# HKPolyU-UAV/FLVIS

Hardware: AMD Instinct MI355X
Metric: frames/sec/node (640×480 stereo+IMU) + ATE vs CPU ref, EuRoC MH_05 (higher is better)
Workload: dtype u8/f32 LK+GFTT, f64 geometry+BA

## Files before the change

flvis_amd/csrc/lk_kernel.hip:

```cpp
#include "dev_common.hpp"
#include "img_kernels.hpp"

namespace flvis {

constexpr int LK_WIN = 31;
constexpr int LK_PS = 40;
constexpr int LK_PROWS = 34;
constexpr int LK_RM = 4;
constexpr int LK_RS = 52;
constexpr int LK_RROWS = 33 + 2 * LK_RM;
constexpr int LK_TC_HDR = 64;
constexpr int LK_TC_LVL = 64 * 24;

typedef short lk_s2 __attribute__((ext_vector_type(2)));
typedef __attribute__((address_space(1))) uint32_t lk_gu32;
typedef uint32_t lk_u4 __attribute__((ext_vector_type(4)));
__device__ __forceinline__ lk_s2 lk_as_s2(uint32_t v) { return __builtin_bit_cast(lk_s2, v); }
__device__ __forceinline__ float lk_uniform(float v) {
  return __builtin_bit_cast(float, __builtin_amdgcn_readfirstlane(__builtin_bit_cast(int, v)));
}
__device__ __forceinline__ long long lk_uniform64(long long v) {
  const uint32_t lo = (uint32_t)__builtin_amdgcn_readfirstlane((int)(uint32_t)v), hi = (uint32_t)__builtin_amdgcn_readfirstlane((int)(v >> 32));
  return (long long)(((unsigned long long)hi << 32) | lo);
}
typedef unsigned short lk_u2 __attribute__((ext_vector_type(2)));
template <int S>
__device__ __forceinline__ lk_s2 lk_pack_shr(int a0, int a1) {
  static_assert(S >= 8 && S <= 16, "bytes 1 and 2 hold bits 8 .. 23");
  const lk_u2 p = __builtin_bit_cast(lk_u2, __builtin_amdgcn_perm((uint32_t)a1, (uint32_t)a0, 0x06050201u));
  return __builtin_bit_cast(lk_s2, (lk_u2)(p >> (unsigned short)(S - 8)));
}

__device__ __forceinline__ bool lk_load_patch(const uint8_t* __restrict__ img, int w, int h, int pitch, int bx, int by, int X0, int Y0,
                                              int nrows, uint8_t* patch) {
  if (X0 >= -bx && Y0 >= -by && X0 + 39 < w + bx && Y0 + nrows <= h + by) {
    const lk_gu32* const base = (const lk_gu32*)(img + (ptrdiff_t)Y0 * pitch + (X0 & ~3));
    const int sh = X0 & 3;
    int r = (int)threadIdx.x / 9, k = (int)threadIdx.x - 9 * r;
    unsigned off = (unsigned)(r * pitch + 4 * k);
    static_assert(LK_PROWS * 9 <= 5 * 64, "five trips");
    const int n = nrows * 9;
    uint32_t lo[5], hi[5];
#pragma unroll
    for (int t = 0; t < 5; t++) {
      const bool on = (int)threadIdx.x + 64 * t < n;
      const unsigned o = on ? off : 0u;
      lo[t] = *(const lk_gu32*)((const __attribute__((address_space(1))) uint8_t*)base + o);
      hi[t] = *(const lk_gu32*)((const __attribute__((address_space(1))) uint8_t*)base + o + 4);
      k += 1;
      const bool wrap = k >= 9;
      k = wrap ? k - 9 : k;
      off += (unsigned)(7 * pitch + 4) + (wrap ? (unsigned)(pitch - 36) : 0u);
    }
#pragma unroll
    for (int t = 0; t < 5; t++) asm volatile("" : "+v"(lo[t]), "+v"(hi[t]));
    r = (int)threadIdx.x / 9;
    k = (int)threadIdx.x - 9 * r;
    unsigned dst = (unsigned)(r * LK_PS + 4 * k);
#pragma unroll
    for (int t = 0; t < 5; t++) {
      if ((int)threadIdx.x + 64 * t < n) *reinterpret_cast<uint32_t*>(patch + dst) = __builtin_amdgcn_alignbyte(hi[t], lo[t], sh);
      k += 1;
      const bool wrap = k >= 9;
      k = wrap ? k - 9 : k;
      dst += (unsigned)(7 * LK_PS + 4) + (wrap ? (unsigned)(LK_PS - 36) : 0u);
    }
    return false;
  }
  for (int i = threadIdx.x; i < nrows * 9; i += 64) {
    int r = i / 9, k = i - r * 9;
    int Y = Y0 + r, X = X0 + 4 * k;
    uint32_t v;
    if (Y >= 0 && Y < h && X >= 0 && X + 3 < w) {
      const uint8_t* row = img + (size_t)Y * pitch;
      int a = X & ~3, sh = X & 3;
      uint32_t lo = *reinterpret_cast<const uint32_t*>(row + a);
      uint32_t hi = sh ? *reinterpret_cast<const uint32_t*>(row + a + 4) : 0u;
      v = __builtin_amdgcn_alignbyte(hi, lo, sh);
    } else {
      const uint8_t* row = img + (size_t)reflect101c(Y, h) * pitch;
      uint32_t b0 = row[reflect101c(X, w)], b1 = row[reflect101c(X + 1, w)], b2 = row[reflect101c(X + 2, w)],
               b3 = row[reflect101c(X + 3, w)];
      v = b0 | (b1 << 8) | (b2 << 16) | (b3 << 24);
    }
    *reinterpret_cast<uint32_t*>(patch + r * LK_PS + 4 * k) = v;
  }
  return true;
}

__device__ __forceinline__ bool lk_load_region(const uint8_t* __restrict__ img, int w, int h, int pitch, int bx, int by, int X0, int Y0,
                                               uint8_t* region) {
  if (X0 >= -bx && Y0 >= -by && X0 + 51 < w + bx && Y0 + LK_RROWS <= h + by) {
    const __attribute__((address_space(1))) uint8_t* const base = (const __attribute__((address_space(1))) uint8_t*)(img + (ptrdiff_t)Y0 * pitch + X0);
    int r = (int)threadIdx.x / 13, k = (int)threadIdx.x - 13 * r;
    unsigned off = (unsigned)(r * pitch + 4 * k);
    static_assert(LK_RS == 52, "the region rows are contiguous in LDS: item i sits at byte 4 i");
    constexpr int N = LK_RROWS * 13, T = (N + 63) / 64;
    uint32_t v[T];
#pragma unroll
    for (int t = 0; t < T; t++) {
      const bool on = 64 * (t + 1) <= N || (int)threadIdx.x + 64 * t < N;
      v[t] = *(const lk_gu32*)(base + (on ? off : 0u));
      k += 12;
      const bool wrap = k >= 13;
      k = wrap ? k - 13 : k;
      off += (unsigned)(4 * pitch + 48) + (wrap ? (unsigned)(pitch - 52) : 0u);
    }
#pragma unroll
    for (int t = 0; t < T; t++) asm volatile("" : "+v"(v[t]));
#pragma unroll
    for (int t = 0; t < T; t++)
      if (64 * (t + 1) <= N || (int)threadIdx.x + 64 * t < N) *reinterpret_cast<uint32_t*>(region + 4 * ((int)threadIdx.x + 64 * t)) = v[t];
    return false;
  }
  for (int i = threadIdx.x; i < LK_RROWS * 13; i += 64) {
    int r = i / 13, k = i - r * 13;
    int Y = Y0 + r, X = X0 + 4 * k;
    uint32_t v;
    if (Y >= 0 && Y < h && X >= 0 && X + 3 < w) {
      v = *reinterpret_cast<const uint32_t*>(img + (size_t)Y * pitch + X);
    } else {
      const uint8_t* row = img + (size_t)reflect101c(Y, h) * pitch;
      uint32_t b0 = row[reflect101c(X, w)], b1 = row[reflect101c(X + 1, w)], b2 = row[reflect101c(X + 2, w)],
               b3 = row[reflect101c(X + 3, w)];
      v = b0 | (b1 << 8) | (b2 << 16) | (b3 << 24);
    }
    *reinterpret_cast<uint32_t*>(region + r * LK_RS + 4 * k) = v;
  }
  return true;
}

#define LK_PAIR(D, K)                                                                                              \
  ((((K)&3) == 3) ? __builtin_amdgcn_perm((D)[((K) >> 2) + 1], (D)[(K) >> 2], 0x0c040c03u)                         \
                  : __builtin_amdgcn_perm(0u, (D)[(K) >> 2], 0x0c000c00u | (uint32_t)((K)&3) | ((uint32_t)(((K)&3) + 1) << 16)))

__device__ __forceinline__ int lk_dot2_bias(lk_s2 a, lk_s2 b, int bias_uniform) {
  int r;
  asm("v_dot2_i32_i16 %0, %1, %2, %3" : "=v"(r) : "v"(a), "v"(b), "s"(bias_uniform));
  return r;
}
__device__ __forceinline__ void lk_wave_sum2_f32(int v1, int v2, float& f1, float& f2) {
  int a = v1 & 0xffff, b = v1 >> 16, c = v2 & 0xffff, d = v2 >> 16;
#define LK_STEP4(CTRL, RM)                                           \
  {                                                                  \
    const int ta = __builtin_amdgcn_update_dpp(0, a, CTRL, RM, 0xf, false); \
    const int tb = __builtin_amdgcn_update_dpp(0, b, CTRL, RM, 0xf, false); \
    const int tc = __builtin_amdgcn_update_dpp(0, c, CTRL, RM, 0xf, false); \
    const int td = __builtin_amdgcn_update_dpp(0, d, CTRL, RM, 0xf, false); \
    a += ta, b += tb, c += tc, d += td;                              \
  }
  LK_STEP4(0xB1, 0xf)
  LK_STEP4(0x4E, 0xf)
  LK_STEP4(0x141, 0xf)
  LK_STEP4(0x140, 0xf)
  LK_STEP4(0x142, 0xa)
  LK_STEP4(0x143, 0xc)
#undef LK_STEP4
  const float g1 = (float)__builtin_fma((double)b, 65536.0, (double)a), g2 = (float)__builtin_fma((double)d, 65536.0, (double)c);
  f1 = __builtin_bit_cast(float, __builtin_amdgcn_readlane(__builtin_bit_cast(int, g1), 63));
  f2 = __builtin_bit_cast(float, __builtin_amdgcn_readlane(__builtin_bit_cast(int, g2), 63));
}

__device__ __forceinline__ void lk_wave_sum3_wide(int v1, int v2, int v3, long long& s1, long long& s2, long long& s3) {
  int a = v1 & 0xffff, b = v1 >> 16, c = v2 & 0xffff, d = v2 >> 16, e = v3 & 0xffff, f = v3 >> 16;
#define LK_STEP6(CTRL, RM)                                                    \
  {                                                                           \
    const int ta = __builtin_amdgcn_update_dpp(0, a, CTRL, RM, 0xf, false);  \
    const int tb = __builtin_amdgcn_update_dpp(0, b, CTRL, RM, 0xf, false);  \
    const int tc = __builtin_amdgcn_update_dpp(0, c, CTRL, RM, 0xf, false);  \
    const int td = __builtin_amdgcn_update_dpp(0, d, CTRL, RM, 0xf, false);  \
    const int te = __builtin_amdgcn_update_dpp(0, e, CTRL, RM, 0xf, false);  \
    const int tf = __builtin_amdgcn_update_dpp(0, f, CTRL, RM, 0xf, false);  \
    a += ta, b += tb, c += tc, d += td, e += te, f += tf;                     \
  }
  LK_STEP6(0xB1, 0xf)
  LK_STEP6(0x4E, 0xf)
  LK_STEP6(0x141, 0xf)
  LK_STEP6(0x140, 0xf)
  LK_STEP6(0x142, 0xa)
  LK_STEP6(0x143, 0xc)
#undef LK_STEP6
  s1 = ((long long)__builtin_amdgcn_readlane(b, 63) << 16) + (long long)__builtin_amdgcn_readlane(a, 63);
  s2 = ((long long)__builtin_amdgcn_readlane(d, 63) << 16) + (long long)__builtin_amdgcn_readlane(c, 63);
  s3 = ((long long)__builtin_amdgcn_readlane(f, 63) << 16) + (long long)__builtin_amdgcn_readlane(e, 63);
}

template <bool INTERIOR>
__device__ __forceinline__ void lk_template(const uint8_t* patch, int lane, int ipx, int ipy, int W, int H, lk_s2 wT, lk_s2 wB,
                                            lk_s2 (&tI)[8], lk_s2 (&tX)[8], lk_s2 (&tY)[8], int& a11, int& a12, int& a22) {
  constexpr int W_BITS = 14;
  const int r = lane >> 1, c0 = (lane & 1) * 16;
  uint32_t d[3][5];
#pragma unroll
  for (int j = 0; j < 3; j++)
#pragma unroll
    for (int k = 0; k < 5; k++) d[j][k] = *reinterpret_cast<const uint32_t*>(patch + (r + j) * LK_PS + c0 + 4 * k);
  uint32_t bits = 0;
  if (!INTERIOR) {
    const int xs = ipx + c0, Y = ipy + r;
    int lo = -xs, hi = W - xs;
    lo = lo < 0 ? 0 : (lo > 18 ? 18 : lo);
    hi = hi < 0 ? 0 : (hi > 18 ? 18 : hi);
    bits = (Y >= 0 && Y < H && hi > lo) ? (((1u << hi) - 1u) & ~((1u << lo) - 1u)) : 0u;
  }
  lk_s2 DX[2][9], DY[2][9];
  {
    lk_s2 T0[10], T1[10];
#pragma unroll
    for (int j = 0; j < 10; j++) {
      const lk_s2 A = __builtin_bit_cast(lk_s2, LK_PAIR(d[0], 2 * j)), B = __builtin_bit_cast(lk_s2, LK_PAIR(d[1], 2 * j)),
                  Cc = __builtin_bit_cast(lk_s2, LK_PAIR(d[2], 2 * j));
      T0[j] = (A + Cc) * (short)3 + B * (short)10;
      T1[j] = Cc - A;
    }
    const int up2 = ((lane + 2) & 63) * 4;
#pragma unroll
    for (int j = 0; j < 9; j++) {
      DX[0][j] = T0[j + 1] - T0[j];
      const lk_s2 T1o = __builtin_bit_cast(lk_s2, __builtin_amdgcn_perm(__builtin_bit_cast(uint32_t, T1[j + 1]),
                                                                       __builtin_bit_cast(uint32_t, T1[j]), 0x05040302u));
      DY[0][j] = (T1[j + 1] + T1[j]) * (short)3 + T1o * (short)10;
      if (!INTERIOR) {
        const uint32_t m = ((bits >> (2 * j)) & 1u ? 0x0000ffffu : 0u) | ((bits >> (2 * j + 1)) & 1u ? 0xffff0000u : 0u);
        DX[0][j] = __builtin_bit_cast(lk_s2, __builtin_bit_cast(uint32_t, DX[0][j]) & m);
        DY[0][j] = __builtin_bit_cast(lk_s2, __builtin_bit_cast(uint32_t, DY[0][j]) & m);
      }
      DX[1][j] = __builtin_bit_cast(lk_s2, __builtin_amdgcn_ds_bpermute(up2, __builtin_bit_cast(int, DX[0][j])));
      DY[1][j] = __builtin_bit_cast(lk_s2, __builtin_amdgcn_ds_bpermute(up2, __builtin_bit_cast(int, DY[0][j])));
    }
  }
  if (r < LK_WIN) {
#pragma unroll
    for (int c2 = 0; c2 < 8; c2++) {
      int iv[2], ix[2], iy[2];
#pragma unroll
      for (int hh = 0; hh < 2; hh++) {
        const int c = 2 * c2 + hh;
        lk_s2 x0, x1, y0, y1;
        if (hh == 0) {
          x0 = DX[0][c2]; x1 = DX[1][c2]; y0 = DY[0][c2]; y1 = DY[1][c2];
        } else {
          x0 = __builtin_bit_cast(lk_s2, __builtin_amdgcn_perm(__builtin_bit_cast(uint32_t, DX[0][c2 + 1]), __builtin_bit_cast(uint32_t, DX[0][c2]), 0x05040302u));
          x1 = __builtin_bit_cast(lk_s2, __builtin_amdgcn_perm(__builtin_bit_cast(uint32_t, DX[1][c2 + 1]), __builtin_bit_cast(uint32_t, DX[1][c2]), 0x05040302u));
          y0 = __builtin_bit_cast(lk_s2, __builtin_amdgcn_perm(__builtin_bit_cast(uint32_t, DY[0][c2 + 1]), __builtin_bit_cast(uint32_t, DY[0][c2]), 0x05040302u));
          y1 = __builtin_bit_cast(lk_s2, __builtin_amdgcn_perm(__builtin_bit_cast(uint32_t, DY[1][c2 + 1]), __builtin_bit_cast(uint32_t, DY[1][c2]), 0x05040302u));
        }
        int ax = lk_dot2_bias(x0, wT, 1 << (W_BITS - 1)), ay = lk_dot2_bias(y0, wT, 1 << (W_BITS - 1));
        int ai = lk_dot2_bias(__builtin_bit_cast(lk_s2, LK_PAIR(d[1], c + 1)), wT, 1 << (W_BITS - 5 - 1));
        ax = __builtin_amdgcn_sdot2(x1, wB, ax, false);
        ay = __builtin_amdgcn_sdot2(y1, wB, ay, false);
        ai = __builtin_amdgcn_sdot2(__builtin_bit_cast(lk_s2, LK_PAIR(d[2], c + 1)), wB, ai, false);
        const bool on = c0 + c < LK_WIN;
        ix[hh] = on ? (ax >> W_BITS) : 0;
        iy[hh] = on ? (ay >> W_BITS) : 0;
        iv[hh] = on ? (ai >> (W_BITS - 5)) : 0;
      }
      tI[c2] = __builtin_bit_cast(lk_s2, __builtin_amdgcn_perm((uint32_t)iv[1], (uint32_t)iv[0], 0x05040100u));
      tX[c2] = __builtin_bit_cast(lk_s2, __builtin_amdgcn_perm((uint32_t)ix[1], (uint32_t)ix[0], 0x05040100u));
      tY[c2] = __builtin_bit_cast(lk_s2, __builtin_amdgcn_perm((uint32_t)iy[1], (uint32_t)iy[0], 0x05040100u));
      a11 = __builtin_amdgcn_sdot2(tX[c2], tX[c2], a11, false);
      a12 = __builtin_amdgcn_sdot2(tX[c2], tY[c2], a12, false);
      a22 = __builtin_amdgcn_sdot2(tY[c2], tY[c2], a22, false);
    }
  } else {
#pragma unroll
    for (int c = 0; c < 8; c++) {
      tI[c] = lk_s2{0, 0};
      tX[c] = lk_s2{0, 0};
      tY[c] = lk_s2{0, 0};
    }
  }
}

__device__ __forceinline__ bool lk_template_level(const uint8_t* img, int W, int H, int pitch, int bx, int by, int ipx, int ipy, int iw00,
                                                  int iw01, int iw10, int iw11, uint8_t* patch, int lane, lk_s2 (&tI)[8], lk_s2 (&tX)[8],
                                                  lk_s2 (&tY)[8], long long& iA11, long long& iA12, long long& iA22) {
  __syncthreads();
  const bool slow = lk_load_patch(img, W, H, pitch, bx, by, ipx - 1, ipy - 1, LK_PROWS, patch);
  __syncthreads();
  int a11 = 0, a12 = 0, a22 = 0;
  const bool interior = ipx >= 0 && ipx + 32 <= W - 1 && ipy >= 0 && ipy + 31 <= H - 1;
  const lk_s2 wT = lk_s2{(short)iw00, (short)iw01}, wB = lk_s2{(short)iw10, (short)iw11};
  if (interior)
    lk_template<true>(patch, lane, ipx, ipy, W, H, wT, wB, tI, tX, tY, a11, a12, a22);
  else
    lk_template<false>(patch, lane, ipx, ipy, W, H, wT, wB, tI, tX, tY, a11, a12, a22);
  lk_wave_sum3_wide(a11, a12, a22, iA11, iA12, iA22);
  return slow;
}
struct LKTmpl {
  uint32_t w[24];
  long long a11, a12, a22;
};
__device__ __noinline__ void lk_template_level_cold(const uint8_t* img, int W, int H, int pitch, int bx, int by, int ipx, int ipy, int iw00,
                                                    int iw01, int iw10, int iw11, uint8_t* patch, int lane, LKTmpl* out) {
  lk_s2 tI[8], tX[8], tY[8];
  long long a11, a12, a22;
  lk_template_level(img, W, H, pitch, bx, by, ipx, ipy, iw00, iw01, iw10, iw11, patch, lane, tI, tX, tY, a11, a12, a22);
#pragma unroll
  for (int k = 0; k < 8; k++) {
    out->w[k] = __builtin_bit_cast(uint32_t, tI[k]);
    out->w[8 + k] = __builtin_bit_cast(uint32_t, tX[k]);
    out->w[16 + k] = __builtin_bit_cast(uint32_t, tY[k]);
  }
  out->a11 = a11;
  out->a12 = a12;
  out->a22 = a22;
}

__device__ __forceinline__ void lk_tc_store_level(uint32_t* tc_ptr, int level, int lane, const lk_s2 (&tI)[8], const lk_s2 (&tX)[8],
                                                  const lk_s2 (&tY)[8], long long iA11, long long iA12, long long iA22) {
  lk_u4* dst = reinterpret_cast<lk_u4*>(tc_ptr + LK_TC_HDR + (size_t)level * LK_TC_LVL) + lane;
  uint32_t wI[8];
#pragma unroll
  for (int k = 0; k < 8; k++) wI[k] = __builtin_bit_cast(uint32_t, tI[k]);
  if (lane == 63) {
    wI[0] = (uint32_t)iA11; wI[1] = (uint32_t)((unsigned long long)iA11 >> 32);
    wI[2] = (uint32_t)iA12; wI[3] = (uint32_t)((unsigned long long)iA12 >> 32);
    wI[4] = (uint32_t)iA22; wI[5] = (uint32_t)((unsigned long long)iA22 >> 32);
  }
#pragma unroll
  for (int k = 0; k < 2; k++) {
    __builtin_nontemporal_store(lk_u4{wI[4 * k], wI[4 * k + 1], wI[4 * k + 2], wI[4 * k + 3]}, dst + 64 * k);
    __builtin_nontemporal_store(lk_u4{__builtin_bit_cast(uint32_t, tX[4 * k]), __builtin_bit_cast(uint32_t, tX[4 * k + 1]),
                                      __builtin_bit_cast(uint32_t, tX[4 * k + 2]), __builtin_bit_cast(uint32_t, tX[4 * k + 3])}, dst + 64 * (2 + k));
    __builtin_nontemporal_store(lk_u4{__builtin_bit_cast(uint32_t, tY[4 * k]), __builtin_bit_cast(uint32_t, tY[4 * k + 1]),
                                      __builtin_bit_cast(uint32_t, tY[4 * k + 2]), __builtin_bit_cast(uint32_t, tY[4 * k + 3])}, dst + 64 * (4 + k));
  }
}

__device__ __forceinline__ const uint8_t* lk_level_ptr(const PyrSel& P, int level, int s, int kc, const uint8_t* ind0) {
  const ImgSel& I = P.lvl[level];
  if (I.ind) return (level == 0 ? ind0 : *I.ind) + (size_t)s * P.stride[level];
  return I.b[I.cur ? (kc ^ I.flip) : 0] + (size_t)s * P.stride[level];
}

#ifndef FLVIS_LK_WAVES
#define FLVIS_LK_WAVES 4
#endif
#ifndef FLVIS_LK_WAVES_T
#define FLVIS_LK_WAVES_T 4
#endif
#ifdef FLVIS_LK_UTIL
__device__ unsigned long long g_lk_wt[3][8][32768][2];
#define LK_UTIL_BEGIN const unsigned long long lk_t0_ = wall_clock64(); const unsigned lk_widx_ = (blockIdx.y * gridDim.x + blockIdx.x) & 32767u;
#define LK_UTIL_END(ROLE)                                                              \
  if (threadIdx.x == 0) {                                                              \
    unsigned long long* u_ = g_lk_wt[(ROLE) % 3][prm.dbg_slot & 7][lk_widx_];          \
    u_[0] = lk_t0_;                                                                    \
    u_[1] = wall_clock64();                                                            \
  }
#else
#define LK_UTIL_BEGIN
#define LK_UTIL_END(ROLE)
#endif
template <int ROLE>
__device__ __forceinline__ void lk_track_body(const PyrSel& prev, const PyrSel& next, const float* __restrict__ prev_pts,
                                              float* __restrict__ next_pts, uint8_t* __restrict__ status,
                                              const int* __restrict__ count, int nmax, const LKParams& prm,
                                              const int* __restrict__ active) {
  int s = blockIdx.y, bx = blockIdx.x;
  {
    const int G = gridDim.x, N = G * gridDim.y;
    if ((N & 7) == 0) {
      const int L = bx + G * s;
      const int Lp = (L & 7) * (N >> 3) + (L >> 3);
      s = Lp / G;
      bx = Lp - s * G;
    }
  }
  if (active && !active[s]) return;
  int n = count[s];
  if (n > nmax) n = nmax;
  if (bx >= n) return;
  LK_UTIL_BEGIN
  __shared__ __attribute__((aligned(16))) uint8_t patch[LK_RROWS * LK_RS + 12];
  const int lane = threadIdx.x;
  int kc_prev = 0, kc_next = 0;
#pragma unroll
  for (int l = LK_MAX_LEVELS - 1; l >= 0; l--) {
    if (l <= prev.levels && prev.lvl[l].cur) kc_prev = prev.lvl[l].cur[s];
    if (l <= next.levels && next.lvl[l].cur) kc_next = next.lvl[l].cur[s];
  }
  const uint8_t* const ind_prev0 = prev.lvl[0].ind ? *prev.lvl[0].ind : nullptr;
  const uint8_t* const ind_next0 = next.lvl[0].ind ? *next.lvl[0].ind : nullptr;
  const int r = lane >> 1;
  const int c0 = (lane & 1) * 16;
  const int W_BITS = 14;
  double eps2 = prm.eps2;
  if (ROLE == 1) asm volatile("" : "+v"(eps2));
  const float FLT_SCALE = 1.f / (1 << 20);
  const float halfWin = (LK_WIN - 1) * 0.5f;

  for (int pb = bx; pb < n; pb += gridDim.x) {
    const int p = prm.order == 1 ? n - 1 - pb : pb;
    const size_t pi = ((size_t)s * nmax + p) * 2;
    const float ppx0 = lk_uniform(prev_pts[pi]), ppy0 = lk_uniform(prev_pts[pi + 1]);
    float nx = lk_uniform(next_pts[pi]), ny = lk_uniform(next_pts[pi + 1]);
    int st = 1;
    uint32_t* tc_ptr = nullptr;
    bool tc_store = false, tc_hit = false;
    uint32_t tc_mask = 0;
    if (ROLE == 2 && prm.tc_mode == 1) {
      if (p < prm.tc_cap) {
        tc_store = true;
        tc_ptr = prm.tc + ((size_t)s * prm.tc_cap + p) * prm.tc_stride;
      }
    } else if (ROLE == 1 && prm.tc_mode == 2) {
      const int code = __builtin_amdgcn_readfirstlane(prm.tc_slot[(size_t)s * nmax + p]);
      if (code >= 0 && (code & 0xffff) < prm.tc_cap) {
        tc_ptr = prm.tc + ((size_t)s * prm.tc_cap + (code & 0xffff)) * prm.tc_stride;
        tc_hit = true;
        tc_mask = (uint32_t)code >> 16;
      }
    }
    lk_u4 pq[6] = {};
    int pq_level = -1;
    for (int level = prev.levels; level >= 0; level--) {
      const float sc = (float)(1. / (1 << level));
      float ppx = ppx0 * sc, ppy = ppy0 * sc;
      float npx, npy;
      if (level == prev.levels) {
        if (prm.use_initial) {
          npx = nx * sc;
          npy = ny * sc;
        } else {
          npx = ppx;
          npy = ppy;
        }
      } else {
        npx = nx * 2.f;
        npy = ny * 2.f;
      }
      nx = npx;
      ny = npy;
      const int W = prev.w[level], H = prev.h[level];
      ppx -= halfWin;
      ppy -= halfWin;
      const int ipx = (int)floorf(ppx), ipy = (int)floorf(ppy);
      if (ipx < -LK_WIN || ipx >= W || ipy < -LK_WIN || ipy >= H) {
        if (level == 0) st = 0;
        continue;
      }
      float a = ppx - (float)ipx, b = ppy - (float)ipy;
      int iw00 = __float2int_rn((1.f - a) * (1.f - b) * (float)(1 << W_BITS));
      int iw01 = __float2int_rn(a * (1.f - b) * (float)(1 << W_BITS));
      int iw10 = __float2int_rn((1.f - a) * b * (float)(1 << W_BITS));
      int iw11 = (1 << W_BITS) - iw00 - iw01 - iw10;

      lk_s2 tI[8], tX[8], tY[8];
      long long iA11, iA12, iA22;
      const bool cached = ROLE == 1 && tc_hit && ((tc_mask >> level) & 1u);
      constexpr bool kEarlyRegion = ROLE == 1;
      int JW = 0, JH = 0;
      const uint8_t* Jimg = nullptr;
      if (kEarlyRegion) {
        JW = next.w[level], JH = next.h[level];
        Jimg = lk_level_ptr(next, level, s, kc_next, ind_next0);
      }
      bool region_ok = false;
      int RX0 = 0, RY0 = 0;
      if (cached) {
        if (prm.stats_tc && lane == 0) atomicAdd(&prm.stats_tc[0], 1ull);
        if (pq_level != level) {
          const lk_u4* src = reinterpret_cast<const lk_u4*>(tc_ptr + LK_TC_HDR + (size_t)level * LK_TC_LVL) + lane;
#pragma unroll
          for (int k = 0; k < 6; k++) pq[k] = __builtin_nontemporal_load(src + 64 * k);
        }
        if (kEarlyRegion) {
        {
          const int einx = (int)floorf(npx - halfWin), einy = (int)floorf(npy - halfWin);
          if (!(einx < -LK_WIN || einx >= JW || einy < -LK_WIN || einy >= JH)) {
            RX0 = (einx - LK_RM) & ~3;
            RY0 = einy - LK_RM;
            __syncthreads();
            const bool slow = lk_load_region(Jimg, JW, JH, next.pitch[level], next.bx[level], next.by[level], RX0, RY0, patch);
            __syncthreads();
            if (prm.stats_tc && slow && lane == 0) atomicAdd(&prm.stats_tc[2], 1ull);
            region_ok = true;
          }
        }
        }
        lk_u4 q[6];
#pragma unroll
        for (int k = 0; k < 6; k++) q[k] = pq[k];
        pq_level = -1;
        iA11 = (long long)(((unsigned long long)(uint32_t)__builtin_amdgcn_readlane((int)q[0].y, 63) << 32) | (uint32_t)__builtin_amdgcn_readlane((int)q[0].x, 63));
        iA12 = (long long)(((unsigned long long)(uint32_t)__builtin_amdgcn_readlane((int)q[0].w, 63) << 32) | (uint32_t)__builtin_amdgcn_readlane((int)q[0].z, 63));
        iA22 = (long long)(((unsigned long long)(uint32_t)__builtin_amdgcn_readlane((int)q[1].y, 63) << 32) | (uint32_t)__builtin_amdgcn_readlane((int)q[1].x, 63));
#pragma unroll
        for (int k = 0; k < 2; k++) {
          tI[4 * k + 0] = lk_as_s2(q[k].x); tI[4 * k + 1] = lk_as_s2(q[k].y);
          tI[4 * k + 2] = lk_as_s2(q[k].z); tI[4 * k + 3] = lk_as_s2(q[k].w);
          tX[4 * k + 0] = lk_as_s2(q[2 + k].x); tX[4 * k + 1] = lk_as_s2(q[2 + k].y);
          tX[4 * k + 2] = lk_as_s2(q[2 + k].z); tX[4 * k + 3] = lk_as_s2(q[2 + k].w);
          tY[4 * k + 0] = lk_as_s2(q[4 + k].x); tY[4 * k + 1] = lk_as_s2(q[4 + k].y);
          tY[4 * k + 2] = lk_as_s2(q[4 + k].z); tY[4 * k + 3] = lk_as_s2(q[4 + k].w);
        }
      } else if (ROLE == 1) {
        LKTmpl T;
        lk_template_level_cold(lk_level_ptr(prev, level, s, kc_prev, ind_prev0), W, H, prev.pitch[level], prev.bx[level], prev.by[level], ipx, ipy, iw00,
                               iw01, iw10, iw11, patch, lane, &T);
#pragma unroll
        for (int k = 0; k < 8; k++) {
          tI[k] = lk_as_s2(T.w[k]);
          tX[k] = lk_as_s2(T.w[8 + k]);
          tY[k] = lk_as_s2(T.w[16 + k]);
        }
        iA11 = lk_uniform64(T.a11);
        iA12 = lk_uniform64(T.a12);
        iA22 = lk_uniform64(T.a22);
      } else {
        const bool slow = lk_template_level(lk_level_ptr(prev, level, s, kc_prev, ind_prev0), W, H, prev.pitch[level], prev.bx[level], prev.by[level], ipx,
                                            ipy, iw00, iw01, iw10, iw11, patch, lane, tI, tX, tY, iA11, iA12, iA22);
        if (prm.stats_tc && slow && lane == 0) atomicAdd(&prm.stats_tc[1], 1ull);
        if (ROLE == 2 && tc_store) {
          lk_tc_store_level(tc_ptr, level, lane, tI, tX, tY, iA11, iA12, iA22);
          tc_mask |= 1u << level;
        }
      }
      const float A11 = (float)iA11 * FLT_SCALE, A12 = (float)iA12 * FLT_SCALE, A22 = (float)iA22 * FLT_SCALE;
      float D = A11 * A22 - A12 * A12;
      const float minEig = __fdiv_rn(A22 + A11 - sqrtf((A11 - A22) * (A11 - A22) + 4.f * A12 * A12),
                                     (float)(2 * LK_WIN * LK_WIN));
      if (minEig < prm.min_eig || D < 1.1920929e-07f) {
        if (level == 0) st = 0;
        continue;
      }
      D = __fdiv_rn(1.f, D);
      npx -= halfWin;
      npy -= halfWin;
      float pdx = 0.f, pdy = 0.f;
      if (!kEarlyRegion) {
        JW = next.w[level], JH = next.h[level];
        Jimg = lk_level_ptr(next, level, s, kc_next, ind_next0);
      }
      int iters_run = 0;
      for (int j = 0; j < prm.max_iter; j++) {
        iters_run = j + 1;
        const int inx = (int)floorf(npx), iny = (int)floorf(npy);
        if ((unsigned)inx + (unsigned)LK_WIN >= (unsigned)(JW + LK_WIN) || (unsigned)iny + (unsigned)LK_WIN >= (unsigned)(JH + LK_WIN)) {
          if (level == 0) st = 0;
          break;
        }
        a = npx - (float)inx;
        b = npy - (float)iny;
        iw00 = __float2int_rn((1.f - a) * (1.f - b) * (float)(1 << W_BITS));
        iw01 = __float2int_rn(a * (1.f - b) * (float)(1 << W_BITS));
        iw10 = __float2int_rn((1.f - a) * b * (float)(1 << W_BITS));
        iw11 = (1 << W_BITS) - iw00 - iw01 - iw10;
        if (!region_ok || (unsigned)(inx - RX0) > 15u || (unsigned)(iny - RY0) > (unsigned)(2 * LK_RM)) {
          RX0 = (inx - LK_RM) & ~3;
          RY0 = iny - LK_RM;
          __syncthreads();
          const bool slow = lk_load_region(Jimg, JW, JH, next.pitch[level], next.bx[level], next.by[level], RX0, RY0, patch);
          __syncthreads();
          if (prm.stats_tc && slow && lane == 0) atomicAdd(&prm.stats_tc[2], 1ull);
          region_ok = true;
        }
        int b1, b2;
        {
          const int bx = inx - RX0 + c0, sh = bx & 3;
          const uint8_t* rp = patch + (iny - RY0 + r) * LK_RS + (bx & ~3);
          uint32_t e[2][5];
#pragma unroll
          for (int q = 0; q < 2; q++) {
            uint32_t dd[6];
#pragma unroll
            for (int k = 0; k < 6; k++) dd[k] = *reinterpret_cast<const uint32_t*>(rp + q * LK_RS + 4 * k);
#pragma unroll
            for (int k = 0; k < 5; k++) e[q][k] = __builtin_amdgcn_alignbyte(dd[k + 1], dd[k], sh);
          }
          const lk_s2 wT = lk_s2{(short)iw00, (short)iw01}, wB = lk_s2{(short)iw10, (short)iw11};
          b1 = 0, b2 = 0;
#pragma unroll
          for (int c2 = 0; c2 < 8; c2++) {
            const int c = 2 * c2;
            int acc0 = lk_dot2_bias(__builtin_bit_cast(lk_s2, LK_PAIR(e[0], c)), wT, 1 << (W_BITS - 5 - 1));
            int acc1 = lk_dot2_bias(__builtin_bit_cast(lk_s2, LK_PAIR(e[0], c + 1)), wT, 1 << (W_BITS - 5 - 1));
            acc0 = __builtin_amdgcn_sdot2(__builtin_bit_cast(lk_s2, LK_PAIR(e[1], c)), wB, acc0, false);
            acc1 = __builtin_amdgcn_sdot2(__builtin_bit_cast(lk_s2, LK_PAIR(e[1], c + 1)), wB, acc1, false);
            const lk_s2 diff = lk_pack_shr<W_BITS - 5>(acc0, acc1) - tI[c2];
            b1 = __builtin_amdgcn_sdot2(diff, tX[c2], b1, false);
            b2 = __builtin_amdgcn_sdot2(diff, tY[c2], b2, false);
          }
        }
        float sb1, sb2;
        lk_wave_sum2_f32(b1, b2, sb1, sb2);
        const float fb1 = sb1 * FLT_SCALE, fb2 = sb2 * FLT_SCALE;
        const float ddx = (A12 * fb2 - A22 * fb1) * D;
        const float ddy = (A12 * fb1 - A11 * fb2) * D;
        npx += ddx;
        npy += ddy;
        nx = npx + halfWin;
        ny = npy + halfWin;
        if (__builtin_amdgcn_ballot_w64((double)ddx * (double)ddx + (double)ddy * (double)ddy <= eps2) != 0) break;
        if (j > 0 && fabs((double)(ddx + pdx)) < 0.01 && fabs((double)(ddy + pdy)) < 0.01) {
          nx -= ddx * 0.5f;
          ny -= ddy * 0.5f;
          break;
        }
        pdx = ddx;
        pdy = ddy;
      }
      if (prm.stats && lane == 0) {
        atomicAdd(&prm.stats[2 * level], (unsigned long long)iters_run);
        atomicAdd(&prm.stats[2 * level + 1], 1ull);
      }
      if (st && level == 0) {
        const float fx = nx - halfWin, fy = ny - halfWin;
        const int inx = (int)floorf(fx), iny = (int)floorf(fy);
        if (inx < -LK_WIN || inx >= JW || iny < -LK_WIN || iny >= JH) st = 0;
      }
    }
    if (lane == 0) {
      next_pts[pi] = nx;
      next_pts[pi + 1] = ny;
      status[(size_t)s * nmax + p] = (uint8_t)st;
      if (ROLE == 2 && tc_store) {
        tc_ptr[0] = __float_as_uint(ppx0);
        tc_ptr[1] = __float_as_uint(ppy0);
        *reinterpret_cast<long long*>(tc_ptr + 2) = prm.tc_tag[s];
        tc_ptr[4] = tc_mask;
      }
    }
  }
  LK_UTIL_END(ROLE)
}

__global__ __launch_bounds__(64) __attribute__((amdgpu_waves_per_eu(FLVIS_LK_WAVES, FLVIS_LK_WAVES))) void k_lk_track(
    PyrSel prev, PyrSel next, const float* __restrict__ prev_pts, float* __restrict__ next_pts, uint8_t* __restrict__ status,
    const int* __restrict__ count, int nmax, LKParams prm, const int* __restrict__ active) {
  lk_track_body<0>(prev, next, prev_pts, next_pts, status, count, nmax, prm, active);
}
__global__ __launch_bounds__(64) __attribute__((amdgpu_waves_per_eu(FLVIS_LK_WAVES_T, FLVIS_LK_WAVES_T))) void k_lk_track_temporal(
    PyrSel prev, PyrSel next, const float* __restrict__ prev_pts, float* __restrict__ next_pts, uint8_t* __restrict__ status,
    const int* __restrict__ count, int nmax, LKParams prm, const int* __restrict__ active) {
  lk_track_body<1>(prev, next, prev_pts, next_pts, status, count, nmax, prm, active);
}
__global__ __launch_bounds__(64) __attribute__((amdgpu_waves_per_eu(FLVIS_LK_WAVES, FLVIS_LK_WAVES))) void k_lk_track_stereo(
    PyrSel prev, PyrSel next, const float* __restrict__ prev_pts, float* __restrict__ next_pts, uint8_t* __restrict__ status,
    const int* __restrict__ count, int nmax, LKParams prm, const int* __restrict__ active) {
  lk_track_body<2>(prev, next, prev_pts, next_pts, status, count, nmax, prm, active);
}

int lk_tc_slot_dwords(int levels) { return LK_TC_HDR + (levels + 1) * LK_TC_LVL; }

void launch_lk_track(hipStream_t st, const PyrSel& prev, const PyrSel& next, const float* prev_pts, float* next_pts,
                     uint8_t* status, const int* count, int nmax, int S, LKParams prm, const int* active, int max_pts, int role) {
  int gx = nmax < 512 ? nmax : 512;
  if (max_pts > 0 && max_pts < gx) gx = (max_pts + 7) & ~7;
  if (gx > nmax) gx = nmax;
  if (role == 1)
    hipLaunchKernelGGL(k_lk_track_temporal, dim3(gx, S), dim3(64), 0, st, prev, next, prev_pts, next_pts, status, count, nmax, prm, active);
  else if (role == 2)
    hipLaunchKernelGGL(k_lk_track_stereo, dim3(gx, S), dim3(64), 0, st, prev, next, prev_pts, next_pts, status, count, nmax, prm, active);
  else
    hipLaunchKernelGGL(k_lk_track, dim3(gx, S), dim3(64), 0, st, prev, next, prev_pts, next_pts, status, count, nmax, prm, active);
}

}

#ifdef FLVIS_LK_UTIL
extern "C" int flvis_debug_lk_util(unsigned long long* out, int reset) {
  const size_t bytes = sizeof(unsigned long long) * 3 * 8 * 32768 * 2;
  if (out && hipMemcpyFromSymbol(out, HIP_SYMBOL(flvis::g_lk_wt), bytes) != hipSuccess) return -1;
  if (reset) {
    void* dp = nullptr;
    if (hipGetSymbolAddress(&dp, HIP_SYMBOL(flvis::g_lk_wt)) != hipSuccess || hipMemset(dp, 0, bytes) != hipSuccess) return -1;
  }
  return 0;
}
#endif
```

Before: 64170.

## Simplify LK patch/region loads, repack pyramid args, cache float Hessian and inverse

The patch and region loaders now compute per-lane offsets once and step by whole row blocks per trip, dropping the per-trip wrap arithmetic. Pyramid selection is repacked on the host into 64-byte per-level records with the buffer flip and the current-slot pointer pre-resolved, so the kernel reads each level's parameters in one scalar load and no longer scans levels for the slot. The template cache now stores the float Hessian, determinant, min eigenvalue and reciprocal determinant, so the temporal tracker skips the conversion, square root and divisions on cache hits. The cost is a larger kernel argument block and a changed cache format that all roles must agree on.

```diff
diff --git a/flvis_amd/csrc/lk_kernel.hip b/flvis_amd/csrc/lk_kernel.hip
--- a/flvis_amd/csrc/lk_kernel.hip
+++ b/flvis_amd/csrc/lk_kernel.hip
@@ -34,37 +34,26 @@
 __device__ __forceinline__ bool lk_load_patch(const uint8_t* __restrict__ img, int w, int h, int pitch, int bx, int by, int X0, int Y0,
                                               int nrows, uint8_t* patch) {
   if (X0 >= -bx && Y0 >= -by && X0 + 39 < w + bx && Y0 + nrows <= h + by) {
-    const lk_gu32* const base = (const lk_gu32*)(img + (ptrdiff_t)Y0 * pitch + (X0 & ~3));
+    const __attribute__((address_space(1))) uint8_t* const base =
+        (const __attribute__((address_space(1))) uint8_t*)(img + (ptrdiff_t)Y0 * pitch + (X0 & ~3));
     const int sh = X0 & 3;
-    int r = (int)threadIdx.x / 9, k = (int)threadIdx.x - 9 * r;
-    unsigned off = (unsigned)(r * pitch + 4 * k);
-    static_assert(LK_PROWS * 9 <= 5 * 64, "five trips");
-    const int n = nrows * 9;
+    static_assert(LK_PROWS <= 5 * 7 && LK_PROWS > 4 * 7, "five trips, and the last one starts on a row of the patch");
+    const int lane = (int)threadIdx.x, r = lane / 9, k = lane - 9 * r;
+    const unsigned off = lane < 63 ? (unsigned)(r * pitch + 4 * k) : 0u;
     uint32_t lo[5], hi[5];
 #pragma unroll
     for (int t = 0; t < 5; t++) {
-      const bool on = (int)threadIdx.x + 64 * t < n;
+      const bool on = lane < 63 && 7 * t + r < nrows;
       const unsigned o = on ? off : 0u;
-      lo[t] = *(const lk_gu32*)((const __attribute__((address_space(1))) uint8_t*)base + o);
-      hi[t] = *(const lk_gu32*)((const __attribute__((address_space(1))) uint8_t*)base + o + 4);
-      k += 1;
-      const bool wrap = k >= 9;
-      k = wrap ? k - 9 : k;
-      off += (unsigned)(7 * pitch + 4) + (wrap ? (unsigned)(pitch - 36) : 0u);
-    }
-#pragma unroll
-    for (int t = 0; t < 5; t++) asm volatile("" : "+v"(lo[t]), "+v"(hi[t]));
-    r = (int)threadIdx.x / 9;
-    k = (int)threadIdx.x - 9 * r;
-    unsigned dst = (unsigned)(r * LK_PS + 4 * k);
-#pragma unroll
-    for (int t = 0; t < 5; t++) {
-      if ((int)threadIdx.x + 64 * t < n) *reinterpret_cast<uint32_t*>(patch + dst) = __builtin_amdgcn_alignbyte(hi[t], lo[t], sh);
-      k += 1;
-      const bool wrap = k >= 9;
-      k = wrap ? k - 9 : k;
-      dst += (unsigned)(7 * LK_PS + 4) + (wrap ? (unsigned)(LK_PS - 36) : 0u);
-    }
+      const __attribute__((address_space(1))) uint8_t* const bt = base + (ptrdiff_t)(7 * t) * pitch;
+      lo[t] = *(const lk_gu32*)(bt + o);
+      hi[t] = *(const lk_gu32*)(bt + o + 4);
+    }
+    asm volatile("" : "+v"(lo[0]), "+v"(hi[0]), "+v"(lo[1]), "+v"(hi[1]), "+v"(lo[2]), "+v"(hi[2]), "+v"(lo[3]), "+v"(hi[3]), "+v"(lo[4]), "+v"(hi[4]));
+    uint8_t* const dst = patch + r * LK_PS + 4 * k;
+#pragma unroll
+    for (int t = 0; t < 5; t++)
+      if (lane < 63 && 7 * t + r < nrows) *reinterpret_cast<uint32_t*>(dst + 7 * LK_PS * t) = __builtin_amdgcn_alignbyte(hi[t], lo[t], sh);
     return false;
   }
   for (int i = threadIdx.x; i < nrows * 9; i += 64) {
@@ -92,25 +81,21 @@
                                                uint8_t* region) {
   if (X0 >= -bx && Y0 >= -by && X0 + 51 < w + bx && Y0 + LK_RROWS <= h + by) {
     const __attribute__((address_space(1))) uint8_t* const base = (const __attribute__((address_space(1))) uint8_t*)(img + (ptrdiff_t)Y0 * pitch + X0);
-    int r = (int)threadIdx.x / 13, k = (int)threadIdx.x - 13 * r;
-    unsigned off = (unsigned)(r * pitch + 4 * k);
-    static_assert(LK_RS == 52, "the region rows are contiguous in LDS: item i sits at byte 4 i");
-    constexpr int N = LK_RROWS * 13, T = (N + 63) / 64;
+    static_assert(LK_RS == 52, "the region rows are contiguous in LDS: a block of four rows is 52 dwords");
+    constexpr int T = (LK_RROWS + 3) / 4, LAST = (LK_RROWS - 4 * (T - 1)) * 13;
+    const int lane = (int)threadIdx.x, r = lane / 13, k = lane - 13 * r;
+    const unsigned off = lane < 52 ? (unsigned)(r * pitch + 4 * k) : 0u;
     uint32_t v[T];
 #pragma unroll
-    for (int t = 0; t < T; t++) {
-      const bool on = 64 * (t + 1) <= N || (int)threadIdx.x + 64 * t < N;
-      v[t] = *(const lk_gu32*)(base + (on ? off : 0u));
-      k += 12;
-      const bool wrap = k >= 13;
-      k = wrap ? k - 13 : k;
-      off += (unsigned)(4 * pitch + 48) + (wrap ? (unsigned)(pitch - 52) : 0u);
-    }
-#pragma unroll
-    for (int t = 0; t < T; t++) asm volatile("" : "+v"(v[t]));
-#pragma unroll
-    for (int t = 0; t < T; t++)
-      if (64 * (t + 1) <= N || (int)threadIdx.x + 64 * t < N) *reinterpret_cast<uint32_t*>(region + 4 * ((int)threadIdx.x + 64 * t)) = v[t];
+    for (int t = 0; t < T; t++) v[t] = *(const lk_gu32*)(base + (ptrdiff_t)(4 * t) * pitch + (t < T - 1 || lane < LAST ? off : 0u));
+    static_assert(T == 11, "the operand list below");
+    asm volatile("" : "+v"(v[0]), "+v"(v[1]), "+v"(v[2]), "+v"(v[3]), "+v"(v[4]), "+v"(v[5]), "+v"(v[6]), "+v"(v[7]), "+v"(v[8]), "+v"(v[9]),
+                 "+v"(v[10]));
+    if (lane < 52) {
+#pragma unroll
+      for (int t = 0; t < T - 1; t++) *reinterpret_cast<uint32_t*>(region + 4 * lane + 4 * LK_RS * t) = v[t];
+      if (lane < LAST) *reinterpret_cast<uint32_t*>(region + 4 * lane + 4 * LK_RS * (T - 1)) = v[T - 1];
+    }
     return false;
   }
   for (int i = threadIdx.x; i < LK_RROWS * 13; i += 64) {
@@ -309,15 +294,14 @@
 }
 
 __device__ __forceinline__ void lk_tc_store_level(uint32_t* tc_ptr, int level, int lane, const lk_s2 (&tI)[8], const lk_s2 (&tX)[8],
-                                                  const lk_s2 (&tY)[8], long long iA11, long long iA12, long long iA22) {
+                                                  const lk_s2 (&tY)[8], float A11, float A12, float A22, float D, float minEig, float invD) {
   lk_u4* dst = reinterpret_cast<lk_u4*>(tc_ptr + LK_TC_HDR + (size_t)level * LK_TC_LVL) + lane;
   uint32_t wI[8];
 #pragma unroll
   for (int k = 0; k < 8; k++) wI[k] = __builtin_bit_cast(uint32_t, tI[k]);
   if (lane == 63) {
-    wI[0] = (uint32_t)iA11; wI[1] = (uint32_t)((unsigned long long)iA11 >> 32);
-    wI[2] = (uint32_t)iA12; wI[3] = (uint32_t)((unsigned long long)iA12 >> 32);
-    wI[4] = (uint32_t)iA22; wI[5] = (uint32_t)((unsigned long long)iA22 >> 32);
+    wI[0] = __float_as_uint(A11); wI[1] = __float_as_uint(A12); wI[2] = __float_as_uint(A22);
+    wI[3] = __float_as_uint(D); wI[4] = __float_as_uint(minEig); wI[5] = __float_as_uint(invD);
   }
 #pragma unroll
   for (int k = 0; k < 2; k++) {
@@ -329,10 +313,38 @@
   }
 }
 
-__device__ __forceinline__ const uint8_t* lk_level_ptr(const PyrSel& P, int level, int s, int kc, const uint8_t* ind0) {
-  const ImgSel& I = P.lvl[level];
-  if (I.ind) return (level == 0 ? ind0 : *I.ind) + (size_t)s * P.stride[level];
-  return I.b[I.cur ? (kc ^ I.flip) : 0] + (size_t)s * P.stride[level];
+struct alignas(64) LKLevel {
+  const uint8_t* b[2];
+  const uint8_t* const* ind;
+  size_t stride;
+  int w, h, pitch, bx, by;
+  int pad_[3];
+};
+static_assert(sizeof(LKLevel) == 64, "one s_load_dwordx16");
+struct alignas(64) LKPyr {
+  LKLevel lvl[LK_MAX_LEVELS];
+  const int* cur;
+  int levels;
+};
+static LKPyr lk_pyr(const PyrSel& P) {
+  LKPyr q{};
+  q.levels = P.levels;
+  for (int l = P.levels < LK_MAX_LEVELS ? P.levels : LK_MAX_LEVELS - 1; l >= 0; l--) {
+    const ImgSel& I = P.lvl[l];
+    LKLevel& V = q.lvl[l];
+    V.b[0] = I.b[I.cur ? (I.flip & 1) : 0];
+    V.b[1] = I.b[I.cur ? ((I.flip & 1) ^ 1) : 0];
+    V.ind = I.ind;
+    V.stride = P.stride[l];
+    V.w = P.w[l], V.h = P.h[l], V.pitch = P.pitch[l], V.bx = P.bx[l], V.by = P.by[l];
+    if (I.cur) q.cur = I.cur;
+  }
+  return q;
+}
+
+__device__ __forceinline__ const uint8_t* lk_level_ptr(const LKLevel& V, int level, int s, int kc, const uint8_t* ind0) {
+  if (V.ind) return (level == 0 ? ind0 : *V.ind) + (size_t)s * V.stride;
+  return (kc ? V.b[1] : V.b[0]) + (size_t)s * V.stride;
 }
 
 #ifndef FLVIS_LK_WAVES
@@ -355,7 +367,7 @@
 #define LK_UTIL_END(ROLE)
 #endif
 template <int ROLE>
-__device__ __forceinline__ void lk_track_body(const PyrSel& prev, const PyrSel& next, const float* __restrict__ prev_pts,
+__device__ __forceinline__ void lk_track_body(const LKPyr& prev, const LKPyr& next, const float* __restrict__ prev_pts,
                                               float* __restrict__ next_pts, uint8_t* __restrict__ status,
                                               const int* __restrict__ count, int nmax, const LKParams& prm,
                                               const int* __restrict__ active) {
@@ -376,12 +388,7 @@
   LK_UTIL_BEGIN
   __shared__ __attribute__((aligned(16))) uint8_t patch[LK_RROWS * LK_RS + 12];
   const int lane = threadIdx.x;
-  int kc_prev = 0, kc_next = 0;
-#pragma unroll
-  for (int l = LK_MAX_LEVELS - 1; l >= 0; l--) {
-    if (l <= prev.levels && prev.lvl[l].cur) kc_prev = prev.lvl[l].cur[s];
-    if (l <= next.levels && next.lvl[l].cur) kc_next = next.lvl[l].cur[s];
-  }
+  const int kc_prev = prev.cur ? prev.cur[s] : 0, kc_next = next.cur ? next.cur[s] : 0;
   const uint8_t* const ind_prev0 = prev.lvl[0].ind ? *prev.lvl[0].ind : nullptr;
   const uint8_t* const ind_next0 = next.lvl[0].ind ? *next.lvl[0].ind : nullptr;
   const int r = lane >> 1;
@@ -417,7 +424,9 @@
     lk_u4 pq[6] = {};
     int pq_level = -1;
     for (int level = prev.levels; level >= 0; level--) {
-      const float sc = (float)(1. / (1 << level));
+      static_assert(LK_MAX_LEVELS <= 126, "2^-level is a normal float");
+      const float sc = __uint_as_float((uint32_t)(127 - level) << 23);
+      const LKLevel PV = prev.lvl[level], NV = next.lvl[level];
       float ppx = ppx0 * sc, ppy = ppy0 * sc;
       float npx, npy;
       if (level == prev.levels) {
@@ -434,7 +443,7 @@
       }
       nx = npx;
       ny = npy;
-      const int W = prev.w[level], H = prev.h[level];
+      const int W = PV.w, H = PV.h;
       ppx -= halfWin;
       ppy -= halfWin;
       const int ipx = (int)floorf(ppx), ipy = (int)floorf(ppy);
@@ -449,14 +458,15 @@
       int iw11 = (1 << W_BITS) - iw00 - iw01 - iw10;
 
       lk_s2 tI[8], tX[8], tY[8];
-      long long iA11, iA12, iA22;
+      long long iA11 = 0, iA12 = 0, iA22 = 0;
+      float A11 = 0.f, A12 = 0.f, A22 = 0.f, D = 0.f, minEig = 0.f, cD = 0.f;
       const bool cached = ROLE == 1 && tc_hit && ((tc_mask >> level) & 1u);
       constexpr bool kEarlyRegion = ROLE == 1;
       int JW = 0, JH = 0;
       const uint8_t* Jimg = nullptr;
       if (kEarlyRegion) {
-        JW = next.w[level], JH = next.h[level];
-        Jimg = lk_level_ptr(next, level, s, kc_next, ind_next0);
+        JW = NV.w, JH = NV.h;
+        Jimg = lk_level_ptr(NV, level, s, kc_next, ind_next0);
       }
       bool region_ok = false;
       int RX0 = 0, RY0 = 0;
@@ -474,7 +484,7 @@
             RX0 = (einx - LK_RM) & ~3;
             RY0 = einy - LK_RM;
             __syncthreads();
-            const bool slow = lk_load_region(Jimg, JW, JH, next.pitch[level], next.bx[level], next.by[level], RX0, RY0, patch);
+            const bool slow = lk_load_region(Jimg, JW, JH, NV.pitch, NV.bx, NV.by, RX0, RY0, patch);
             __syncthreads();
             if (prm.stats_tc && slow && lane == 0) atomicAdd(&prm.stats_tc[2], 1ull);
             region_ok = true;
@@ -485,9 +495,12 @@
 #pragma unroll
         for (int k = 0; k < 6; k++) q[k] = pq[k];
         pq_level = -1;
-        iA11 = (long long)(((unsigned long long)(uint32_t)__builtin_amdgcn_readlane((int)q[0].y, 63) << 32) | (uint32_t)__builtin_amdgcn_readlane((int)q[0].x, 63));
-        iA12 = (long long)(((unsigned long long)(uint32_t)__builtin_amdgcn_readlane((int)q[0].w, 63) << 32) | (uint32_t)__builtin_amdgcn_readlane((int)q[0].z, 63));
-        iA22 = (long long)(((unsigned long long)(uint32_t)__builtin_amdgcn_readlane((int)q[1].y, 63) << 32) | (uint32_t)__builtin_amdgcn_readlane((int)q[1].x, 63));
+        A11 = __uint_as_float((uint32_t)__builtin_amdgcn_readlane((int)q[0].x, 63));
+        A12 = __uint_as_float((uint32_t)__builtin_amdgcn_readlane((int)q[0].y, 63));
+        A22 = __uint_as_float((uint32_t)__builtin_amdgcn_readlane((int)q[0].z, 63));
+        D = __uint_as_float((uint32_t)__builtin_amdgcn_readlane((int)q[0].w, 63));
+        minEig = __uint_as_float((uint32_t)__builtin_amdgcn_readlane((int)q[1].x, 63));
+        cD = __uint_as_float((uint32_t)__builtin_amdgcn_readlane((int)q[1].y, 63));
 #pragma unroll
         for (int k = 0; k < 2; k++) {
           tI[4 * k + 0] = lk_as_s2(q[k].x); tI[4 * k + 1] = lk_as_s2(q[k].y);
@@ -499,7 +512,7 @@
         }
       } else if (ROLE == 1) {
         LKTmpl T;
-        lk_template_level_cold(lk_level_ptr(prev, level, s, kc_prev, ind_prev0), W, H, prev.pitch[level], prev.bx[level], prev.by[level], ipx, ipy, iw00,
+        lk_template_level_cold(lk_level_ptr(PV, level, s, kc_prev, ind_prev0), W, H, PV.pitch, PV.bx, PV.by, ipx, ipy, iw00,
                                iw01, iw10, iw11, patch, lane, &T);
 #pragma unroll
         for (int k = 0; k < 8; k++) {
@@ -511,29 +524,37 @@
         iA12 = lk_uniform64(T.a12);
         iA22 = lk_uniform64(T.a22);
       } else {
-        const bool slow = lk_template_level(lk_level_ptr(prev, level, s, kc_prev, ind_prev0), W, H, prev.pitch[level], prev.bx[level], prev.by[level], ipx,
+        const bool slow = lk_template_level(lk_level_ptr(PV, level, s, kc_prev, ind_prev0), W, H, PV.pitch, PV.bx, PV.by, ipx,
                                             ipy, iw00, iw01, iw10, iw11, patch, lane, tI, tX, tY, iA11, iA12, iA22);
         if (prm.stats_tc && slow && lane == 0) atomicAdd(&prm.stats_tc[1], 1ull);
-        if (ROLE == 2 && tc_store) {
-          lk_tc_store_level(tc_ptr, level, lane, tI, tX, tY, iA11, iA12, iA22);
-          tc_mask |= 1u << level;
-        }
-      }
-      const float A11 = (float)iA11 * FLT_SCALE, A12 = (float)iA12 * FLT_SCALE, A22 = (float)iA22 * FLT_SCALE;
-      float D = A11 * A22 - A12 * A12;
-      const float minEig = __fdiv_rn(A22 + A11 - sqrtf((A11 - A22) * (A11 - A22) + 4.f * A12 * A12),
-                                     (float)(2 * LK_WIN * LK_WIN));
-      if (minEig < prm.min_eig || D < 1.1920929e-07f) {
+      }
+      float invD = 0.f;
+      if (!cached) {
+        A11 = (float)iA11 * FLT_SCALE, A12 = (float)iA12 * FLT_SCALE, A22 = (float)iA22 * FLT_SCALE;
+        D = A11 * A22 - A12 * A12;
+        minEig = __fdiv_rn(A22 + A11 - sqrtf((A11 - A22) * (A11 - A22) + 4.f * A12 * A12), (float)(2 * LK_WIN * LK_WIN));
+      }
+      const bool skip = minEig < prm.min_eig || D < 1.1920929e-07f;
+      if (cached) {
+        invD = cD;
+      } else if (!skip) {
+        invD = __fdiv_rn(1.f, D);
+      }
+      if (ROLE == 2 && tc_store) {
+        lk_tc_store_level(tc_ptr, level, lane, tI, tX, tY, A11, A12, A22, D, minEig, invD);
+        tc_mask |= 1u << level;
+      }
+      if (skip) {
         if (level == 0) st = 0;
         continue;
       }
-      D = __fdiv_rn(1.f, D);
+      D = invD;
       npx -= halfWin;
       npy -= halfWin;
       float pdx = 0.f, pdy = 0.f;
       if (!kEarlyRegion) {
-        JW = next.w[level], JH = next.h[level];
-        Jimg = lk_level_ptr(next, level, s, kc_next, ind_next0);
+        JW = NV.w, JH = NV.h;
+        Jimg = lk_level_ptr(NV, level, s, kc_next, ind_next0);
       }
       int iters_run = 0;
       for (int j = 0; j < prm.max_iter; j++) {
@@ -553,7 +574,7 @@
           RX0 = (inx - LK_RM) & ~3;
           RY0 = iny - LK_RM;
           __syncthreads();
-          const bool slow = lk_load_region(Jimg, JW, JH, next.pitch[level], next.bx[level], next.by[level], RX0, RY0, patch);
+          const bool slow = lk_load_region(Jimg, JW, JH, NV.pitch, NV.bx, NV.by, RX0, RY0, patch);
           __syncthreads();
           if (prm.stats_tc && slow && lane == 0) atomicAdd(&prm.stats_tc[2], 1ull);
           region_ok = true;
@@ -629,28 +650,29 @@
 }
 
 __global__ __launch_bounds__(64) __attribute__((amdgpu_waves_per_eu(FLVIS_LK_WAVES, FLVIS_LK_WAVES))) void k_lk_track(
-    PyrSel prev, PyrSel next, const float* __restrict__ prev_pts, float* __restrict__ next_pts, uint8_t* __restrict__ status,
+    LKPyr prev, LKPyr next, const float* __restrict__ prev_pts, float* __restrict__ next_pts, uint8_t* __restrict__ status,
     const int* __restrict__ count, int nmax, LKParams prm, const int* __restrict__ active) {
   lk_track_body<0>(prev, next, prev_pts, next_pts, status, count, nmax, prm, active);
 }
 __global__ __launch_bounds__(64) __attribute__((amdgpu_waves_per_eu(FLVIS_LK_WAVES_T, FLVIS_LK_WAVES_T))) void k_lk_track_temporal(
-    PyrSel prev, PyrSel next, const float* __restrict__ prev_pts, float* __restrict__ next_pts, uint8_t* __restrict__ status,
+    LKPyr prev, LKPyr next, const float* __restrict__ prev_pts, float* __restrict__ next_pts, uint8_t* __restrict__ status,
     const int* __restrict__ count, int nmax, LKParams prm, const int* __restrict__ active) {
   lk_track_body<1>(prev, next, prev_pts, next_pts, status, count, nmax, prm, active);
 }
 __global__ __launch_bounds__(64) __attribute__((amdgpu_waves_per_eu(FLVIS_LK_WAVES, FLVIS_LK_WAVES))) void k_lk_track_stereo(
-    PyrSel prev, PyrSel next, const float* __restrict__ prev_pts, float* __restrict__ next_pts, uint8_t* __restrict__ status,
+    LKPyr prev, LKPyr next, const float* __restrict__ prev_pts, float* __restrict__ next_pts, uint8_t* __restrict__ status,
     const int* __restrict__ count, int nmax, LKParams prm, const int* __restrict__ active) {
   lk_track_body<2>(prev, next, prev_pts, next_pts, status, count, nmax, prm, active);
 }
 
 int lk_tc_slot_dwords(int levels) { return LK_TC_HDR + (levels + 1) * LK_TC_LVL; }
 
-void launch_lk_track(hipStream_t st, const PyrSel& prev, const PyrSel& next, const float* prev_pts, float* next_pts,
+void launch_lk_track(hipStream_t st, const PyrSel& prev_sel, const PyrSel& next_sel, const float* prev_pts, float* next_pts,
                      uint8_t* status, const int* count, int nmax, int S, LKParams prm, const int* active, int max_pts, int role) {
   int gx = nmax < 512 ? nmax : 512;
   if (max_pts > 0 && max_pts < gx) gx = (max_pts + 7) & ~7;
   if (gx > nmax) gx = nmax;
+  const LKPyr prev = lk_pyr(prev_sel), next = lk_pyr(next_sel);
   if (role == 1)
     hipLaunchKernelGGL(k_lk_track_temporal, dim3(gx, S), dim3(64), 0, st, prev, next, prev_pts, next_pts, status, count, nmax, prm, active);
   else if (role == 2)
```

After: 65630 (median of 6 runs). +2.3%, better.
